# XuZerui2023/Radar-Signal-Simulation-and-Target-Detection

Measured on AMD Instinct MI355X. Metric: frames/sec + range-Doppler cells/sec, 16ch×8beam×4096samp×128pulse, higher is better.
Workload: dtype fp64 (complex128); 1 GPU; BASELINE config #2: x2 C=16 B=8 N=4096 P=128 G=2811; frames_per_launch=8, ring=8, parallelism=frame-sharded x1, used_samples=3027, targets_reported=258400

## Files before the change

include/rsp.h:

```cpp
#ifndef RSP_H
#define RSP_H

#include <stddef.h>
#include <stdint.h>

#ifdef __cplusplus
extern "C" {
#endif

#define RSP_ABI_VERSION 4

typedef enum rsp_status {
    RSP_OK = 0,
    RSP_ERR_INVALID = -1,
    RSP_ERR_UNSUPPORTED = -2,
    RSP_ERR_DEVICE = -3,
    RSP_ERR_NOMEM = -4,
    RSP_ERR_OVERFLOW = -5
} rsp_status;

typedef enum rsp_dtype {
    RSP_C64 = 1,
    RSP_C128 = 2
} rsp_dtype;
// ... 145 lines not shown
    int32_t Ls, ntaps, delay;
    int32_t Lh, M, V;
    int32_t nblocks;
    int32_t rows_per_wg;
} rsp_k2_segment;
typedef struct rsp_k2_layout {
    int32_t k2_pts;
    int32_t wg_per_cu;
    int32_t NZ;
    int32_t nseg, njobs;
    int32_t nwg;
    rsp_k2_segment seg[3];
} rsp_k2_layout;
int32_t rsp_query_k2_layout(const rsp_plan* plan, rsp_k2_layout* out);

int32_t rsp_plan_describe(const rsp_sig_config* cfg, const rsp_cfar_params* cfar,
                          const rsp_cluster_params* cluster, const rsp_precomputed* pre,
                          const rsp_plan_options* opt, int32_t ncu, rsp_sizes* sizes, rsp_k1_route* route);
int32_t rsp_plan_describe_k3(const rsp_sig_config* cfg, const rsp_cfar_params* cfar,
                             const rsp_cluster_params* cluster, const rsp_precomputed* pre,
                             const rsp_plan_options* opt, int32_t ncu, rsp_k3_tiling* tiling);
int32_t rsp_plan_describe_k2(const rsp_sig_config* cfg, const rsp_cfar_params* cfar,
                             const rsp_cluster_params* cluster, const rsp_precomputed* pre,
                             const rsp_plan_options* opt, int32_t ncu, rsp_k2_layout* layout);

int32_t rsp_process_cube(rsp_plan* plan, const void* cube, int32_t dtype, int32_t layout,
                         int32_t frame_idx, rsp_frame_out* out);

int32_t rsp_last_detections(const rsp_plan* plan, rsp_detection* dets, int32_t cap, int32_t* n);
int32_t rsp_last_targets(const rsp_plan* plan, rsp_target* targets, int32_t cap, int32_t* n);

int32_t rsp_process_targets(rsp_plan* plan, const rsp_target_in* targets, int32_t n_targets,
                            int32_t frame_idx, uint64_t seed, double p_noise, rsp_frame_out* out);

int32_t rsp_synthesize_device(rsp_plan* plan, const rsp_target_in* targets, int32_t n_targets,
                              int32_t frame_idx, uint64_t seed, double p_noise, void* d_cube);
int32_t rsp_profile_synthesis(rsp_plan* plan, const rsp_target_in* targets, int32_t n_targets, int32_t iters,
                              void* d_cube, float* ms_out, int64_t* bytes_out);

// ... 248 lines not shown
```

radar-signal-simulation-and-target-detection_amd/csrc/rsp_geometry.cpp:

```cpp
#include "rsp_geometry.h"

#include <algorithm>
#include <cmath>
#include <cstdint>
#include <utility>

__attribute__((visibility("hidden"))) int rsp_set_error(int code, const char* fmt, ...);

namespace {

template <class... A>
int fail(int code, const char* fmt, A... a) { return rsp_set_error(code, fmt, a...); }

using cd = std::complex<double>;

bool is_pow2(int x) { return x > 0 && (x & (x - 1)) == 0; }
int ilog2i(int x) { int l = 0; while ((1 << l) < x) ++l; return l; }
size_t cplx_bytes(const Geometry& g) { return g.prec == RSP_PREC_F64 ? 16 : 8; }

void fft_d(std::vector<cd>& a, int sign) {
    const int n = (int)a.size();
    if (!is_pow2(n)) {
        std::vector<cd> o(n);
        for (int k = 0; k < n; ++k) {
// ... 329 lines not shown
    for (const Unit& u : units) {
        int x = 0;
        for (int c = 1; c < 8; ++c)
            if (q[c].size() < q[x].size()) x = c;
        q[x].insert(q[x].end(), u.wgs.begin(), u.wgs.end());
    }
    std::vector<int>& order = h.k2order;
    size_t qmax = 0;
    for (auto& v : q) qmax = std::max(qmax, v.size());
    for (size_t sl = 0; sl < qmax; ++sl)
        for (int x = 0; x < 8; ++x)
            if (sl < q[x].size()) order.push_back(q[x][sl]);
    for (int w : single) order.push_back(w);
    if ((int)order.size() != g.nwg_k2)
        return fail(RSP_ERR_INVALID, "K2 dispatch order covers %d of %d workgroups", (int)order.size(), g.nwg_k2);
    return RSP_OK;
}

#define RSP_K3_TILE_KB 48
#define RSP_K3_RT_C128 32
int derive_k3_tiling(Geometry& g) {
    const size_t rsz = cplx_bytes(g) / 2;
    g.cfar_hR = (std::max(g.refR + g.guardR, 2) + 3) & ~3;
    g.cfar_RT = rsz == 4 ? 64 : RSP_K3_RT_C128;
    const bool k3_nohalo = k3_fast_params(g);
    const int hx = k3_nohalo ? 0 : 2;
    g.cfar_W = ((g.cfar_RT + hx * g.cfar_hR + 3) & ~3) + (rsz == 8 ? 2 : 0);
    const int hV = g.refV + g.guardV, ncut = std::max(g.P - 2 * hV, 1);
    const int hrows = k3_nohalo ? 0 : 2 * hV;
    const int rows_max = (int)((RSP_K3_TILE_KB * 1024) / ((size_t)g.cfar_W * rsz));
// ... 259 lines not shown
    return RSP_OK;
}

extern "C" int32_t rsp_plan_describe_k2(const rsp_sig_config* cfg, const rsp_cfar_params* cfar, const rsp_cluster_params* cluster,
                                        const rsp_precomputed* pre, const rsp_plan_options* opt, int32_t ncu,
                                        rsp_k2_layout* layout) {
    int rc = rsp_plan_check_args(cfg, cfar, cluster, pre, opt);
    if (rc) return rc;
    PlanHost h;
    if ((rc = rsp_plan_derive(cfg, cfar, cluster, pre, opt, ncu, &h))) return rc;
    const int32_t gates[RSP_MAX_SEG] = {pre->N_gate_narrow, pre->N_gate_medium, pre->N_gate_long};
    if (layout) rsp_fill_k2_layout(h.g, gates, layout);
    return RSP_OK;
}

int rsp_stage3_derive(int P, const int32_t* gates, const rsp_stage3_cfar_params* prm, S3Desc* out) {
    if (!gates || !prm || !out) return fail(RSP_ERR_INVALID, "null argument");
    const int64_t G = (int64_t)gates[0] + gates[1] + gates[2];
    if (P < 1 || gates[0] < 0 || gates[1] < 0 || gates[2] < 0 || G < 1 || G > INT32_MAX)
        return fail(RSP_ERR_INVALID, "bad map shape P=%d segments %d, %d, %d", P, gates[0], gates[1], gates[2]);
    const int r = prm->refCells_R, s = prm->saveCells_R;
    if (r < 1 || s < 0) return fail(RSP_ERR_INVALID, "bad CFAR window refCells_R=%d saveCells_R=%d (r >= 1, s >= 0)", r, s);
    if (prm->CFARmethod_R != 0 && prm->CFARmethod_R != 1)
        return fail(RSP_ERR_INVALID, "CFARmethod_R must be 0 (greatest of) or 1 (smallest of), got %d", prm->CFARmethod_R);
    if (prm->MTD_0v_num < 0) return fail(RSP_ERR_INVALID, "MTD_0v_num must be >= 0, got %d", prm->MTD_0v_num);
    if (!std::isfinite(prm->T_CFAR) || prm->T_CFAR <= 0) return fail(RSP_ERR_INVALID, "T_CFAR must be finite and > 0, got %g", prm->T_CFAR);
    const int64_t H = (int64_t)r + s;
    if (H > RSP_S3_HMAX)
        return fail(RSP_ERR_INVALID, "CFAR window refCells_R + saveCells_R = %lld exceeds the kernel's tile halo %d", (long long)H,
                    RSP_S3_HMAX);
// ... 86 lines not shown
```

radar-signal-simulation-and-target-detection_amd/csrc/rsp_geometry.h:

```cpp
#pragma once
#include "rsp.h"

#include <complex>
#include <stddef.h>
#include <stdint.h>
#include <vector>

#ifdef __HIPCC__
#define RSP_HD __host__ __device__
#else
#define RSP_HD
#endif

#define RSP_MAX_F 8
#define RSP_K2_POINTS 4096
#define RSP_K2_MIXPTS 2560
#define K1_THREADS 512

#define RSP_PREC_F32 0
#define RSP_PREC_F64 1

constexpr size_t RSP_LDS_BYTES = 160 * 1024;

struct SegDesc {
    int type;
    int ga, gb;
    int seg_lo;
    int lo, hi;
    int off;
    int ntaps, delay, Ls, taps_off;
    int Lh, M, logM, V, nblocks, H_off, tw_off;
    int rows_per_wg;
};

struct K2Job {
    int seg, blk, wg_begin, wg_count;
};

#define RSP_MAX_SEG 3
#define RSP_MAX_JOBS 16
#define RSP_MAX_IVL 4

struct Geometry {
    int prec;
    int C, B, P, N, G;
    int cpitch;
    int Gp;
    int NT, nU, ntiles, Ppad;
    int NZ, nzc;
    int twPp_elems;
    int pow2P, logP;
// ... 1 lines not shown
    int nseg, njobs, nwg_k2;
    int k2_pts;
    int cfar_RT, cfar_hR, cfar_W;
    int cfar_VB, cfar_nband, cfar_rows;
    int refR, guardR, refV, guardV;
    double T;
    int max_dets;
    int ncu;
    int k1_tiled;
    int mono_c;
    int nivl, ivl_lo[RSP_MAX_IVL], ivl_start[RSP_MAX_IVL];
    SegDesc segs[RSP_MAX_SEG];
    K2Job jobs[RSP_MAX_JOBS];
};
static_assert(sizeof(SegDesc) == 76 && sizeof(K2Job) == 16 && sizeof(Geometry) == 680, "kernel-argument layout");

RSP_HD inline bool k3_fast_params(const Geometry& g) {
    return g.refR == 5 && g.refV == 5 && g.guardR == 10 && g.guardV == 10 && (g.cfar_RT == 32 || g.cfar_RT == 64);
}

RSP_HD inline int k3_ntiles(const Geometry& g) {
    const int rc0 = g.refR + g.guardR;
    return (g.G - rc0 - (rc0 & ~3) + g.cfar_RT - 1) / g.cfar_RT;
}

RSP_HD inline long long k3_map_bytes(const Geometry& g, int real_bytes) {
    if (k3_fast_params(g)) {
        const int hV = g.refV + g.guardV, c0 = (g.refR + g.guardR) & ~3;
        const int rows = g.P - 2 * hV > 0 ? g.P - 2 * hV : 0;
        const int c1 = c0 + k3_ntiles(g) * g.cfar_RT < g.G ? c0 + k3_ntiles(g) * g.cfar_RT : g.G;
// ... 98 lines not shown
size_t mtd_cols_lds(const Geometry& g);

struct PlanHost {
    typedef std::complex<double> cd;
    Geometry g{};
    std::vector<SegDesc> segs;
    std::vector<K2Job> jobs;
    int det_bound = 1;
    size_t z_elems = 0, rdm_elems = 0, mag_elems = 0;
    std::vector<double> atab;
    std::vector<cd> twP, twPp, twD, twQ;
    std::vector<double> win, taps;
    std::vector<cd> H, twM;
    std::vector<double> range_axis, velocity_axis, beam_angles, klut;
    std::vector<int> k2order;
};

#define RSP_S3_CH 256
#define RSP_S3_ROWS 16
#define RSP_S3_HMAX 64
struct S3Desc {
    int P, G;
    int seg_a[3], seg_n[3];
    int r, s, H;
    int method;
    int z0, z1;
    double T;
};
int rsp_stage3_derive(int P, const int32_t* gates, const rsp_stage3_cfar_params* prm, S3Desc* out);

// ... 6 lines not shown
    int method;
    double T;
};
RSP_HD constexpr size_t vc_lds_bytes(int halo, size_t rs) { return (size_t)(RSP_VC_ROWS + 2 * halo) * RSP_VC_COLS * rs; }
int rsp_vcfar_derive(int P, int G, const rsp_vcfar_params* prm, VcDesc* out);

int rsp_plan_check_args(const rsp_sig_config* cfg, const rsp_cfar_params* cfar, const rsp_cluster_params* cluster,
                        const rsp_precomputed* pre, const rsp_plan_options* opt);
int rsp_plan_derive(const rsp_sig_config* cfg, const rsp_cfar_params* cfar, const rsp_cluster_params* cluster,
                    const rsp_precomputed* pre, const rsp_plan_options* opt, int ncu, PlanHost* out);

void rsp_fill_sizes(const Geometry& g, int det_bound, rsp_sizes* s);
void rsp_fill_k1_route(const Geometry& g, rsp_k1_route* out);
void rsp_fill_k3_tiling(const Geometry& g, rsp_k3_tiling* out);
void rsp_fill_k2_layout(const Geometry& g, const int32_t gates[RSP_MAX_SEG], rsp_k2_layout* out);
```

radar-signal-simulation-and-target-detection_amd/csrc/rsp_internal.h:

```cpp
#pragma once
#include <hip/hip_runtime.h>
#include <stdint.h>

#include "rsp_geometry.h"
#include "rsp_music_geometry.h"

#define RSP_LANES 4
#define RSP_NLANES 3
#define K2_THREADS 256
#define RSP_THREADS 256

__device__ __forceinline__ void rsp_philox10(uint32_t c[4], uint32_t k0, uint32_t k1) {
    const uint32_t M0 = 0xD2511F53u, M1 = 0xCD9E8D57u;
#pragma unroll
    for (int r = 0; r < 10; ++r) {
        const uint64_t p0 = (uint64_t)M0 * c[0];
        const uint64_t p1 = (uint64_t)M1 * c[2];
        const uint32_t hi0 = (uint32_t)(p0 >> 32), lo0 = (uint32_t)p0;
        const uint32_t hi1 = (uint32_t)(p1 >> 32), lo1 = (uint32_t)p1;
        const uint32_t n0 = hi1 ^ c[1] ^ k0, n2 = hi0 ^ c[3] ^ k1;
        c[0] = n0; c[1] = lo1; c[2] = n2; c[3] = lo0;
        k0 += 0x9E3779B9u;
        k1 += 0xBB67AE85u;
    }
// ... 13 lines not shown
    unsigned long long* trace;
    DevDet* dets[RSP_MAX_F];
    int* count[RSP_MAX_F];
};

struct DevConsts {
    const void* Atab;
    const void* win;
    const void* twP;
    const void* twPp;
    const void* twD;
    const void* twQ;
    const void* taps;
    const void* H;
    const void* twM;
    const int* k2order;
    const double* range_axis;
    const double* velocity_axis;
    const double* beam_angles;
    const double* klut;
    double deltaR, deltaV;
};

hipError_t launch_k1(const Geometry& g, const DevConsts& k, const FramePtrs& fp, int nf, int mode, hipStream_t s);
hipError_t launch_stream_copy(const void* in, void* out, size_t n16, int ncu, hipStream_t s);
hipError_t launch_k2(const Geometry& g, const DevConsts& k, const FramePtrs& fp, int nf, int rows, hipStream_t s);
hipError_t launch_k3(const Geometry& g, const DevConsts& k, const FramePtrs& fp, int nf, hipStream_t s);
hipError_t launch_mtd_cols(const Geometry& g, const DevConsts& k, const void* pc, void* rdm, hipStream_t s);
hipError_t launch_synth(const Geometry& g, const double* tx, const SynthTargets& tg, int nt, void* tab, int frame_idx,
                        uint64_t seed, double noise_scale, void* cube, hipStream_t s);
hipError_t launch_s3(const S3Desc& d, int prec, bool cplx, const void* in, int n_maps, double* amp, double* thr,
// ... 9 lines not shown
```

radar-signal-simulation-and-target-detection_amd/csrc/rsp_kernels.hip:

```cpp
#include "rsp_internal.h"
#include "rsp_cmag.h"
#include "rsp_noise_math.h"
#include <math.h>
#include <algorithm>

namespace {

typedef float f32x4 __attribute__((ext_vector_type(4)));
typedef double f64x4 __attribute__((ext_vector_type(4)));
typedef unsigned int u32x2 __attribute__((ext_vector_type(2)));
typedef unsigned int u32x4 __attribute__((ext_vector_type(4)));

template <class T> struct CxT;
template <> struct CxT<float> { typedef f2 V; };
template <> struct CxT<double> { typedef d2 V; };
template <class T> using cx = typename CxT<T>::V;
template <class V> struct ScalT;
template <> struct ScalT<f2> { typedef float S; };
template <> struct ScalT<d2> { typedef double S; };
template <class V> using scal = typename ScalT<V>::S;

__device__ __forceinline__ f2 vmul(f2 a, f2 b) { return a.xx * b + a.yy * f2{-b.y, b.x}; }
__device__ __forceinline__ d2 vmul(d2 a, d2 b) { return d2{a.x * b.x - a.y * b.y, a.x * b.y + a.y * b.x}; }
template <bool INV>
// ... 221 lines not shown
template <bool INV, class V> struct Dft<12, INV, V> {
    static __device__ __forceinline__ void run(V* a) { dft_pfa<4, 3, INV>(a); }
};

template <int SH>
__device__ __forceinline__ int lidx(int i) { return SH ? i + (i >> SH) : i; }

template <class V>
struct StoreLds {
    V* buf;
    __device__ __forceinline__ void put(int, int, int, int loff, V x) const { buf[loff] = x; }
};
template <class St> struct StoresLds { static constexpr bool value = false; };
template <class V> struct StoresLds<StoreLds<V>> { static constexpr bool value = true; };

template <int R, bool INV, bool CMP, int NS, class V, class TW>
__device__ __forceinline__ void load_tw(const TW& twk, V (&w)[R]) {
    if constexpr (!CMP) {
#pragma unroll
        for (int r = 1; r < R; ++r) {
            const V t = twk[r - 1];
            w[r] = V{t.x, INV ? -t.y : t.y};
        }
    } else {
        constexpr int lgR = clog2(R - 1) + 1;
        V b[lgR];
#pragma unroll
        for (int i = 0; i < lgR; ++i) {
            const V t = twk[i * NS];
            b[i] = V{t.x, INV ? -t.y : t.y};
        }
#pragma unroll
        for (int r = 1; r < R; ++r) {
            const int hb = 1 << clog2(r);
            w[r] = (hb == r) ? b[clog2(r)] : vmul(w[hb], w[r - hb]);
        }
    }
}

template <int SH, int D, int R>
constexpr bool lidx_sep() {
    constexpr int p = 1 << SH;
    return SH == 0 || D % p == 0 || (p % D == 0 && ((D * R) % p == 0 || p % (D * R) == 0));
}
template <int SH, int D>
constexpr int lidx_off(int r) {
    return r * D + (SH ? (r * D) >> SH : 0);
}

template <int R, bool INV, int NB, int SH, int NTHR, int L, int NS, bool CMP = false, int XL = 0, class V, class TW>
__device__ __forceinline__ void sh_load(const V* buf, int rs, int nrows, const TW& tw, V (&v)[NB][R],
// ... 2 lines not shown
    static_assert(!XL || nb % 128 == 0, "XOR-swizzled input needs r nb to keep the swizzle bits");
    constexpr bool SEP = lidx_sep<SH, nb, R>();
    const int total = nb * nrows;
#pragma unroll
    for (int t = 0; t < NB; ++t) {
        const int beta = tix + t * NTHR;
        if (beta < total) {
            const int row = beta / nb, j = beta - row * nb;
            const V* src = XL ? buf + row * L + (j ^ ((j >> 4) & 7)) : buf + row * rs + (SEP ? lidx<SH>(j) : 0);
            V w[R];
            if (NS > 1) load_tw<R, INV, CMP, NS>(tw + (CMP ? j % NS : (j % NS) * tw_row(R, CMP)), w);
#pragma unroll
            for (int r = 0; r < R; ++r) {
                V x = XL ? src[r * nb] : (SEP ? src[lidx_off<SH, nb>(r)] : src[lidx<SH>(j + r * nb)]);
                if (r > 0 && NS > 1) x = vmul(x, w[r]);
                v[t][r] = x;
            }
        }
    }
}

template <int R, bool INV, int NB, int SH, int NTHR, int L, int NS, int XL = 0, class V, class St>
__device__ __forceinline__ void sh_store(V (&v)[NB][R], int rs, int nrows, const St& st, int tix = threadIdx.x) {
    constexpr int nb = L / R;
    static_assert(!XL || (NS == 1 && R == 16), "XOR-swizzled output: Ns = 1 radix-16 passes");
    const int total = nb * nrows;
#pragma unroll
    for (int t = 0; t < NB; ++t) {
        const int beta = tix + t * NTHR;
        if (beta < total) {
// ... 795 lines not shown
}

template <class T> constexpr int k2_sh() { return RSP_K2_SH; }
constexpr int K2_NOPAD_SH = 30;
template <class T, bool NOPAD> constexpr int k2_sh_np() { return NOPAD ? K2_NOPAD_SH : k2_sh<T>(); }

constexpr int k2_tw_lds(RadixPlan p) {
    return plan_tw_total(p, true) + (plan_is_palindrome(p) ? 0 : plan_tw_total(plan_rev(p), true));
}
constexpr int k2_tw_lds_max() {
    int m = k2_tw_lds(plan_os_2560());
    for (int lg = 6; lg <= 11; ++lg) m = k2_tw_lds(plan_os_pow2(lg)) > m ? k2_tw_lds(plan_os_pow2(lg)) : m;
    return m;
}

template <class T, int SH>
__device__ __forceinline__ void k2_epilogue(const cx<T>* L, int rs, int rows, int row0, int rows_total, int Lh1, int g0,
                                            int gend, cx<T>* __restrict__ rdm, T* __restrict__ mag, int G, int Gp) {
    typedef cx<T> V;
    const int nkeep = gend - g0;
    for (int r = 0; r < rows; ++r) {
        const int rho = row0 + r;
        if (rho >= rows_total) break;
        const V* src = L + r * rs + Lh1;
        const int pad0 = SH ? Lh1 : 0;
        const __amdgpu_buffer_rsrc_t mr = buf_rsrc(mag + (size_t)rho * Gp + g0, (unsigned)nkeep * (unsigned)sizeof(T));
        if (rdm) {
            const __amdgpu_buffer_rsrc_t rr = buf_rsrc(rdm + (size_t)rho * G + g0, (unsigned)nkeep * (unsigned)sizeof(V));
            for (int e = threadIdx.x; e < nkeep; e += K2_THREADS) {
                const V x = src[e + (SH ? ((pad0 + e) >> SH) : 0)];
                buf_st<RSP_RDM_AUX>(rr, (unsigned)e * (unsigned)sizeof(V), x);
                buf_st1(mr, (unsigned)e * (unsigned)sizeof(T), cmag(x));
            }
        } else {
            for (int e = threadIdx.x; e < nkeep; e += K2_THREADS)
                buf_st1(mr, (unsigned)e * (unsigned)sizeof(T), cmag(src[e + (SH ? ((pad0 + e) >> SH) : 0)]));
        }
    }
}

template <int R, int S, class V>
__device__ __forceinline__ void k2_apply_h(V (&x)[R], __amdgpu_buffer_rsrc_t hr, int j) {
    asm volatile("" ::: "memory");
    V h[R];
#pragma unroll
    for (int r = 0; r < R; ++r) h[r] = buf_ld<V>(hr, (unsigned)(j + r * S) * (unsigned)sizeof(V));
#pragma unroll
    for (int r = 0; r < R; ++r) x[r] = vmul(x[r], h[r]);
}

template <bool LDS, class V>
// ... 161 lines not shown
    if (tid < nb0 * rows) {
        const ZWin zw = zrow_window(g, z, row0 + rl, rows_total, off, lo, hi);
        k2_load_wrow<nb0>(g, zw, a + j - lo + off, v0[0]);
        if constexpr (!EPI) {
            const __amdgpu_buffer_rsrc_t hr = buf_rsrc(H + sd.H_off, (unsigned)(M * sizeof(V)));
#pragma unroll
            for (int r = 0; r < R0; ++r)
                hreg[0][r] = buf_ld<V>(hr, (unsigned)(j + r * nb0) * (unsigned)sizeof(V));
        }
    }
    V* twL = L + k2_lds_data(g.k2_pts, SH);
    if constexpr (!NOPAD) stage_lds<K2_THREADS>(twL, twl, NTWF);
    const auto twF = k2_tw_src<!NOPAD, V>(twL, twl);
    const auto twI = twF;
    constexpr int XZ = R0 == 16 ? 1 : 0;
    sh_store<R0, false, NB0, SH, K2_THREADS, M, 1, XZ>(v0, rs, rows, StoreLds<V>{L}, tid);
    __syncthreads();
    K2_STAMP(1);
    sh_pass<R1, false, NB1, SH, K2_THREADS, M, NS1, CMP, XZ>(L, rs, rows, twF, StoreLds<V>{L});
    K2_STAMP(2);
    {
        V v[NB0][R0];
        sh_load<R0, false, NB0, SH, K2_THREADS, M, NS2, CMP>(L, rs, rows, twF + TW2, v, tid);
        __syncthreads();
        const __amdgpu_buffer_rsrc_t hr = buf_rsrc(H + sd.H_off, (unsigned)(M * sizeof(V)));
#pragma unroll
        for (int t = 0; t < NB0; ++t) {
            Dft<R0, false, V>::run(v[t]);
            if constexpr (EPI) {
                k2_apply_h<R0, nb0>(v[t], hr, j);
            } else {
#pragma unroll
                for (int r = 0; r < R0; ++r) v[t][r] = vmul(v[t][r], hreg[t][r]);
            }
        }
        sh_store<R0, true, NB0, SH, K2_THREADS, M, 1, XZ>(v, rs, rows, StoreLds<V>{L}, tid);
        __syncthreads();
    }
    K2_STAMP(3);
    sh_pass<R1, true, NB1, SH, K2_THREADS, M, NS1, CMP, XZ>(L, rs, rows, twI, StoreLds<V>{L});
    K2_STAMP(4);
    const int gend = min(sd.gb, g0 + sd.V);
    if constexpr (EPI) {
        sh_pass<R0, true, NB0, SH, K2_THREADS, M, NS2, CMP>(L, rs, rows, twI + TW2, StoreLds<V>{L});
        k2_epilogue<T, SH>(L, rs, rows, row0, rows_total, Lh1, g0, gend, rdm, mag, G, g.Gp);
    } else {
        static_assert(EPI || (rows == 1 && NS2 == nb0), "last pass: thread j's outputs are j + r NS2 of one row");
        V v[NB0][R0];
        sh_load<R0, true, NB0, SH, K2_THREADS, M, NS2, CMP>(L, rs, rows, twI + TW2, v, tid);
        if (rdm)
            sh_store<R0, true, NB0, SH, K2_THREADS, M, NS2>(
                v, rs, rows, StoreRowK<V, true, NS2, R0>(rdm, mag, G, g.Gp, row0, rows_total, Lh1, g0, gend), tid);
        else
            sh_store<R0, true, NB0, SH, K2_THREADS, M, NS2>(
                v, rs, rows, StoreRowK<V, false, NS2, R0>(rdm, mag, G, g.Gp, row0, rows_total, Lh1, g0, gend), tid);
    }
}

template <class T, int WGS>
__global__ __launch_bounds__(K2_THREADS, WGS) void k2_pc(Geometry g, DevConsts k, FramePtrs fp, int rows_total) {
    constexpr bool EPI = WGS >= 3;
    constexpr bool NOPAD = WGS == 4;
    typedef cx<T> V;
    V* L = reinterpret_cast<V*>(rsp_lds);
    const int f = blockIdx.y;
    const int wg = k.k2order[blockIdx.x];
    int ji = 0;
    while (ji + 1 < g.njobs && wg >= g.jobs[ji + 1].wg_begin) ++ji;
    const K2Job job = g.jobs[ji];
    const SegDesc& sd = g.segs[job.seg];
    const int rows = sd.rows_per_wg;
    const int row0 = (wg - job.wg_begin) * rows;
    const V* __restrict__ z = static_cast<const V*>(fp.z[f]);
    V* __restrict__ rdm = static_cast<V*>(fp.rdm[f]);
    T* __restrict__ mag = static_cast<T*>(fp.mag[f]);
    const int P = g.P, G = g.G;
    const int lo = sd.lo, hi = sd.hi, off = sd.off;
    const int tid = threadIdx.x;
    K2_STAMP(0);
    K2_TAG((unsigned long long)(sd.type * 16 + sd.logM));

    if (sd.type == 1 && sd.logM == 0) {
        k2_fft_job_mix<T, 2560, 16, 10, EPI, NOPAD>(g, k, sd, job, z, rdm, mag, row0, rows_total, L);
    } else if (sd.type == 1) {
        constexpr int PTS = WGS >= 3 ? 2048 : RSP_K2_POINTS;
        constexpr int LGTOP = WGS >= 3 ? 11 : 12;
        switch (sd.logM) {
// ... 814 lines not shown
```

radar-signal-simulation-and-target-detection_amd/csrc/rsp_plan.cpp:

```cpp
#include "rsp.h"
#include "rsp_frame_host.h"
#include "rsp_internal.h"

#include <algorithm>
#include <cmath>
#include <complex>
#include <cstdarg>
#include <cstdio>
#include <cstring>
#include <cstdlib>
#include <condition_variable>
#include <deque>
#include <functional>
#include <memory>
#include <mutex>
#include <string>
#include <thread>
#include <vector>

__attribute__((visibility("hidden"))) void rsp_cluster_frame(const rsp_cluster_params& cp, std::vector<rsp_detection>& dets,
                                                             std::vector<rsp_target>& final_targets);

namespace {

// ... 98 lines not shown
    DevConsts k{};
    rsp_cluster_params cl{};
    SynthConsts sc{};
    int F = 1;
    int det_bound = 1;
    size_t esz = 16;
    size_t rsz = 8;
    size_t z_elems = 0, rdm_elems = 0, mag_elems = 0;
    std::vector<void*> dev_allocs;
    double* d_tx = nullptr;
    double* d_stab = nullptr;
    void* d_cube = nullptr;
    void* d_aux = nullptr;
    void* d_smap = nullptr;
    int32_t gates[3] = {0, 0, 0};
    bool aux_valid = false;
    struct DevBuf {
        void* p = nullptr;
        size_t cap = 0;
    };
    DevBuf s3_in, s3_amp, s3_thr, s3_flags, s3_hits, s3_count;
    unsigned char* h_stage = nullptr;
    size_t h_stage_bytes = 0;
    Lane lanes[RSP_LANES];
    int nlanes = RSP_NLANES;
    int next_lane = 0;
    bool time_stages = false;
    double stage_ms[3] = {0, 0, 0};
    int64_t stage_launches = 0, stage_frames = 0;
    const void* pend_in[RSP_MAX_F];
// ... 541 lines not shown
    rsp_plan* p = new rsp_plan();
    auto bail = [&](int rc) { delete p; return rc; };
    p->device = device;
    p->F = opt->frames_per_launch;
    p->cl = *cluster;
    p->sc = SynthConsts{cfg->c, cfg->fs, cfg->wavelength, cfg->element_spacing, cfg->prt, pre->P_signal_unscaled};
    p->esz = opt->precision == RSP_C128 ? 16 : 8;
    p->rsz = p->esz / 2;
    p->g = h.g;
    p->det_bound = h.det_bound;
    p->z_elems = h.z_elems; p->rdm_elems = h.rdm_elems; p->mag_elems = h.mag_elems;
    p->gates[0] = pre->N_gate_narrow; p->gates[1] = pre->N_gate_medium; p->gates[2] = pre->N_gate_long;

    DevConsts& k = p->k;
    double *dra, *dva, *dang, *dkl;
    int* dord;
    if ((rc = p->upload_r(&k.Atab, h.atab)) || (rc = p->upload_c(&k.twP, h.twP)) || (rc = p->upload_c(&k.twPp, h.twPp)) ||
        (rc = p->upload_c(&k.twD, h.twD)) || (rc = p->upload_c(&k.twQ, h.twQ)) || (rc = p->upload_r(&k.win, h.win)) ||
        (rc = p->upload_r(&k.taps, h.taps)) || (rc = p->upload_c(&k.H, h.H)) || (rc = p->upload_c(&k.twM, h.twM)) ||
        (rc = p->upload(&dra, h.range_axis)) || (rc = p->upload(&dva, h.velocity_axis)) ||
        (rc = p->upload(&dang, h.beam_angles)) || (rc = p->upload(&dkl, h.klut)) || (rc = p->upload(&dord, h.k2order)))
        return bail(rc);
    k.range_axis = dra; k.velocity_axis = dva; k.beam_angles = dang; k.klut = dkl;
    k.k2order = dord;
    k.deltaR = pre->deltaR; k.deltaV = pre->deltaV;
    const Geometry& g = p->g;
    if (pre->tx_pulse) {
        std::vector<double> tx(pre->tx_pulse, pre->tx_pulse + 2 * (size_t)g.N);
        if ((rc = p->upload(&p->d_tx, tx))) return bail(rc);
    }
    if ((rc = p->dalloc(&p->d_stab, (size_t)2 * RSP_MAX_SYNTH_TARGETS * (g.P + g.C)))) return bail(rc);
    if ((rc = p->dalloc_bytes(&p->d_cube, (size_t)std::max(g.C, g.B) * g.cpitch * p->esz))) return bail(rc);
    for (auto& L : p->lanes)
        if ((rc = setup_lane(p, L))) return bail(rc);
    *out = p;
    return RSP_OK;
}

int32_t rsp_set_stage_timing(rsp_plan* p, int32_t on) {
// ... 27 lines not shown
    if (!p || !out) return fail(RSP_ERR_INVALID, "null argument");
    rsp_fill_k1_route(p->g, out);
    return RSP_OK;
}

int32_t rsp_query_k3_tiling(const rsp_plan* p, rsp_k3_tiling* out) {
    if (!p || !out) return fail(RSP_ERR_INVALID, "null argument");
    rsp_fill_k3_tiling(p->g, out);
    return RSP_OK;
}

int32_t rsp_query_k2_layout(const rsp_plan* p, rsp_k2_layout* out) {
    if (!p || !out) return fail(RSP_ERR_INVALID, "null argument");
    rsp_fill_k2_layout(p->g, p->gates, out);
    return RSP_OK;
}

int32_t rsp_process_cube(rsp_plan* p, const void* cube, int32_t dtype, int32_t layout, int32_t frame_idx,
                         rsp_frame_out* out) {
    if (!p || !cube) return fail(RSP_ERR_INVALID, "null argument");
    if (layout != RSP_LAYOUT_PNC) return fail(RSP_ERR_UNSUPPORTED, "layout %d", layout);
    HIPCHK(hipSetDevice(p->device));
    int rc = drain_all(p);
    if (rc) return rc;
    if ((rc = upload_cube(p, cube, dtype, p->g.C, p->d_cube, p->lanes[0].stream))) return rc;
    return run_sync_frame(p, p->d_cube, frame_idx, out);
}

static int synth_into(rsp_plan* p, const rsp_target_in* t, int nt, int frame_idx, uint64_t seed, double p_noise,
                      void* d_cube, hipStream_t s, bool sync) {
// ... 521 lines not shown
```

radar-signal-simulation-and-target-detection_amd/rsp/_abi.py:

```python
import ctypes as ct
import os

LIB_PATH = os.path.join(os.path.dirname(os.path.abspath(__file__)), 'librsp.so')
_INTREE = LIB_PATH

RSP_OK, RSP_ERR_INVALID, RSP_ERR_UNSUPPORTED, RSP_ERR_DEVICE, RSP_ERR_NOMEM, RSP_ERR_OVERFLOW = 0, -1, -2, -3, -4, -5
RSP_C64, RSP_C128 = 1, 2
RSP_LAYOUT_PNC = 0

_dp = ct.POINTER(ct.c_double)


class SigConfig(ct.Structure):
    _fields_ = [('c', ct.c_double), ('fs', ct.c_double), ('fc', ct.c_double), ('prt', ct.c_double),
                ('wavelength', ct.c_double), ('element_spacing', ct.c_double),
                ('prtNum', ct.c_int32), ('point_PRT', ct.c_int32), ('channel_num', ct.c_int32),
                ('beam_num', ct.c_int32)]


class CfarParams(ct.Structure):
    _fields_ = [('refCells_V', ct.c_int32), ('guardCells_V', ct.c_int32), ('refCells_R', ct.c_int32),
                ('guardCells_R', ct.c_int32), ('T_CFAR', ct.c_double)]


# ... 49 lines not shown


class K3Tiling(ct.Structure):
    _fields_ = [('fast', ct.c_int32), ('RT', ct.c_int32), ('hR', ct.c_int32), ('W', ct.c_int32),
                ('n_tiles', ct.c_int32), ('n_bands', ct.c_int32), ('VB', ct.c_int32), ('rows', ct.c_int32)]


class K2Segment(ct.Structure):
    _fields_ = [(n, ct.c_int32) for n in ('present', 'type', 'ga', 'gb', 'seg_lo', 'lo', 'hi', 'Ls', 'ntaps', 'delay',
                                          'Lh', 'M', 'V', 'nblocks', 'rows_per_wg')]


class K2Layout(ct.Structure):
    _fields_ = [('k2_pts', ct.c_int32), ('wg_per_cu', ct.c_int32), ('NZ', ct.c_int32), ('nseg', ct.c_int32),
                ('njobs', ct.c_int32), ('nwg', ct.c_int32), ('seg', K2Segment * 3)]


class Stage3CfarParams(ct.Structure):
    _fields_ = [('refCells_R', ct.c_int32), ('saveCells_R', ct.c_int32), ('CFARmethod_R', ct.c_int32),
                ('MTD_0v_num', ct.c_int32), ('T_CFAR', ct.c_double)]


class Stage3Hit(ct.Structure):
    _fields_ = [('v_idx', ct.c_int32), ('r_idx', ct.c_int32), ('beam_idx', ct.c_int32), ('reserved', ct.c_int32),
                ('amp', ct.c_double), ('threshold', ct.c_double)]


class Stage3Info(ct.Structure):
    _fields_ = [('P', ct.c_int32), ('G', ct.c_int32), ('seg_first', ct.c_int32 * 3), ('seg_len', ct.c_int32 * 3),
                ('notch_first', ct.c_int32), ('notch_last', ct.c_int32), ('halo', ct.c_int32),
# ... 94 lines not shown
    'rsp_plan_options_default': (ct.c_int32, [ct.POINTER(PlanOptions)]),
    'rsp_plan_destroy': (ct.c_int32, [_P]),
    'rsp_query_sizes': (ct.c_int32, [_P, ct.POINTER(Sizes)]),
    'rsp_query_k1_route': (ct.c_int32, [_P, ct.POINTER(K1Route)]),
    'rsp_plan_describe': (ct.c_int32, [ct.POINTER(SigConfig), ct.POINTER(CfarParams), ct.POINTER(ClusterParams),
                                       ct.POINTER(Precomputed), ct.POINTER(PlanOptions), ct.c_int32, ct.POINTER(Sizes),
                                       ct.POINTER(K1Route)]),
    'rsp_query_k3_tiling': (ct.c_int32, [_P, ct.POINTER(K3Tiling)]),
    'rsp_plan_describe_k3': (ct.c_int32, [ct.POINTER(SigConfig), ct.POINTER(CfarParams), ct.POINTER(ClusterParams),
                                          ct.POINTER(Precomputed), ct.POINTER(PlanOptions), ct.c_int32,
                                          ct.POINTER(K3Tiling)]),
    'rsp_query_k2_layout': (ct.c_int32, [_P, ct.POINTER(K2Layout)]),
    'rsp_plan_describe_k2': (ct.c_int32, [ct.POINTER(SigConfig), ct.POINTER(CfarParams), ct.POINTER(ClusterParams),
                                          ct.POINTER(Precomputed), ct.POINTER(PlanOptions), ct.c_int32,
                                          ct.POINTER(K2Layout)]),
    'rsp_process_cube': (ct.c_int32, [_P, _P, ct.c_int32, ct.c_int32, ct.c_int32, ct.POINTER(FrameOut)]),
    'rsp_process_targets': (ct.c_int32, [_P, ct.POINTER(TargetIn), ct.c_int32, ct.c_int32, ct.c_uint64,
                                         ct.c_double, ct.POINTER(FrameOut)]),
    'rsp_synthesize_device': (ct.c_int32, [_P, ct.POINTER(TargetIn), ct.c_int32, ct.c_int32, ct.c_uint64,
                                           ct.c_double, _P]),
    'rsp_profile_synthesis': (ct.c_int32, [_P, ct.POINTER(TargetIn), ct.c_int32, ct.c_int32, _P,
                                           ct.POINTER(ct.c_float), ct.POINTER(ct.c_int64)]),
    'rsp_enqueue_device': (ct.c_int32, [_P, _P, ct.c_int32]),
    'rsp_enqueue_device_n': (ct.c_int32, [_P, ct.POINTER(_P), ct.POINTER(ct.c_int32), ct.c_int32]),
    'rsp_enqueue_device_rdm': (ct.c_int32, [_P, _P, ct.c_int32, _P]),
    'rsp_enqueue_device_rdm_n': (ct.c_int32, [_P, ct.POINTER(_P), ct.POINTER(ct.c_int32), ct.POINTER(_P), ct.c_int32]),
    'rsp_enqueue_host': (ct.c_int32, [_P, _P, ct.c_int32, ct.c_int32]),
    'rsp_host_alloc': (ct.c_int32, [_P, ct.c_int64, ct.POINTER(_P)]),
    'rsp_host_free': (ct.c_int32, [_P, _P]),
    'rsp_process_targets_multi': (ct.c_int32, [ct.POINTER(_P), ct.c_int32, ct.POINTER(ct.POINTER(TargetIn)),
# ... 110 lines not shown
```

radar-signal-simulation-and-target-detection_amd/rsp/plan.py:

```python
import ctypes as ct
import numpy as np

from . import _abi
from ._abi import check, lib


def _dptr(a):
    return a.ctypes.data_as(ct.POINTER(ct.c_double))


def _complex_arg(a):
    c64 = np.asarray(a).dtype == np.complex64
    a = np.asfortranarray(a, None if c64 else np.complex128)
    return a, a.ctypes.data_as(ct.c_void_p), _abi.RSP_C64 if c64 else _abi.RSP_C128


def _gate_cols_arg(gate_cols):
    return (ct.c_int32 * 6)(*[int(x) for fl in gate_cols for x in fl])


def _with_hits(call, first_cap, hits_cap, want_hits):
    cap = (int(hits_cap) if hits_cap is not None else first_cap) if want_hits else 0
    hits = np.zeros(max(cap, 1), HIT_DTYPE)
    total = call(cap, hits.ctypes.data_as(ct.POINTER(_abi.Stage3Hit)) if cap else None, True)
# ... 102 lines not shown
    segs = [{k: getattr(s, k) for k, _ in _abi.K2Segment._fields_ if k != 'present'} if s.present else None
            for s in L.seg]
    return dict(k2_pts=L.k2_pts, wg_per_cu=L.wg_per_cu, NZ=L.NZ, nseg=L.nseg, njobs=L.njobs, nwg=L.nwg, segments=segs)


def describe_k2(config, cfar_params, cluster_params, precomputed_data, precision='c128', k1_tiled=False, ncu=256):
    keep = []
    cfg, cfar, cluster, pre = _marshal(config, cfar_params, cluster_params, precomputed_data, keep)
    opt = _options(0, 1, precision, k1_tiled, 'amplitude')
    L = _abi.K2Layout()
    check(lib().rsp_plan_describe_k2(ct.byref(cfg), ct.byref(cfar), ct.byref(cluster), ct.byref(pre), ct.byref(opt),
                                     int(ncu), ct.byref(L)))
    return _k2_dict(L)


HIT_DTYPE = np.dtype([('v_idx', np.int32), ('r_idx', np.int32), ('beam_idx', np.int32), ('reserved', np.int32),
                      ('amp', np.float64), ('threshold', np.float64)])
STAGE3_WANT = ('mtd', 'amp', 'flags', 'threshold', 'hits')


def _stage3_params(cfar):
    return _abi.Stage3CfarParams(refCells_R=int(cfar['refCells_R']), saveCells_R=int(cfar['saveCells_R']),
                                 CFARmethod_R=int(cfar['CFARmethod_R']), MTD_0v_num=int(cfar['MTD_0v_num']),
                                 T_CFAR=float(cfar['T_CFAR']))


def describe_stage3(P, segments, cfar):
    n1, n2, n3 = (int(x) for x in segments)
    cfg = _abi.SigConfig(prtNum=int(P))
    pre = _abi.Precomputed(N_gate_narrow=n1, N_gate_medium=n2, N_gate_long=n3, N_total_gate=n1 + n2 + n3)
# ... 57 lines not shown

    def k1_route(self):
        r = _abi.K1Route()
        check(lib().rsp_query_k1_route(self.h, ct.byref(r)))
        return _route_dict(r)

    def k3_tiling(self):
        t = _abi.K3Tiling()
        check(lib().rsp_query_k3_tiling(self.h, ct.byref(t)))
        return _tiling_dict(t)

    def k2_layout(self):
        L = _abi.K2Layout()
        check(lib().rsp_query_k2_layout(self.h, ct.byref(L)))
        return _k2_dict(L)

    def _frame_out(self, want_rdm, want_cfar):
        o = _abi.FrameOut()
        bufs = {}
        if want_rdm:
            bufs['rdm'] = np.empty((self.P, self.G, self.B), np.complex128, order='F')
            o.rdm = bufs['rdm'].ctypes.data_as(ct.POINTER(ct.c_double))
        if want_cfar and self.B > 1:
            bufs['cfar'] = np.empty((self.P, self.G, self.B - 1), np.float64, order='F')
            o.cfar_maps = _dptr(bufs['cfar'])
        o.dets, o.dets_cap, o.targets, o.targets_cap = None, 0, None, 0
        return o, bufs, None, None

    def last_detections(self):
        n = ct.c_int32()
# ... 352 lines not shown
```

Baseline: 17850 frames/s.

## Precompute K2 workgroup records, prefetch twiddles across barriers, unroll epilogue stores

K2's per-workgroup job lookup, which walked the job table, is replaced by a host-precomputed 16-byte record (segment, block, first row) read once per workgroup. In the no-pad path, twiddle base values for the next FFT pass are fetched from global memory before the preceding LDS store and barrier, then expanded in registers, so the loads overlap the sync. The epilogue loop that writes magnitudes and RDM is unrolled by four, with loads batched ahead of stores. These raise register pressure through the held twiddle buffers and add query APIs for the records.

```diff
diff --git a/include/rsp.h b/include/rsp.h
--- a/include/rsp.h
+++ b/include/rsp.h
@@ -183,6 +183,14 @@
 } rsp_k2_layout;
 int32_t rsp_query_k2_layout(const rsp_plan* plan, rsp_k2_layout* out);
 
+typedef struct rsp_k2_record {
+    int32_t seg;
+    int32_t blk;
+    int32_t row0;
+    int32_t wg;
+} rsp_k2_record;
+int32_t rsp_query_k2_records(const rsp_plan* plan, rsp_k2_record* out, int32_t cap, int32_t* n);
+
 int32_t rsp_plan_describe(const rsp_sig_config* cfg, const rsp_cfar_params* cfar,
                           const rsp_cluster_params* cluster, const rsp_precomputed* pre,
                           const rsp_plan_options* opt, int32_t ncu, rsp_sizes* sizes, rsp_k1_route* route);
@@ -192,6 +200,10 @@
 int32_t rsp_plan_describe_k2(const rsp_sig_config* cfg, const rsp_cfar_params* cfar,
                              const rsp_cluster_params* cluster, const rsp_precomputed* pre,
                              const rsp_plan_options* opt, int32_t ncu, rsp_k2_layout* layout);
+int32_t rsp_plan_describe_k2_records(const rsp_sig_config* cfg, const rsp_cfar_params* cfar,
+                                     const rsp_cluster_params* cluster, const rsp_precomputed* pre,
+                                     const rsp_plan_options* opt, int32_t ncu, rsp_k2_record* out, int32_t cap,
+                                     int32_t* n);
 
 int32_t rsp_process_cube(rsp_plan* plan, const void* cube, int32_t dtype, int32_t layout,
                          int32_t frame_idx, rsp_frame_out* out);
diff --git a/radar-signal-simulation-and-target-detection_amd/csrc/rsp_geometry.cpp b/radar-signal-simulation-and-target-detection_amd/csrc/rsp_geometry.cpp
--- a/radar-signal-simulation-and-target-detection_amd/csrc/rsp_geometry.cpp
+++ b/radar-signal-simulation-and-target-detection_amd/csrc/rsp_geometry.cpp
@@ -367,6 +367,13 @@
     for (int w : single) order.push_back(w);
     if ((int)order.size() != g.nwg_k2)
         return fail(RSP_ERR_INVALID, "K2 dispatch order covers %d of %d workgroups", (int)order.size(), g.nwg_k2);
+    h.k2rec.reserve(order.size());
+    for (int wg : order) {
+        size_t ji = 0;
+        while (ji + 1 < h.jobs.size() && wg >= h.jobs[ji + 1].wg_begin) ++ji;
+        const K2Job& jb = h.jobs[ji];
+        h.k2rec.push_back(K2Rec{jb.seg, jb.blk, (wg - jb.wg_begin) * h.segs[jb.seg].rows_per_wg, wg});
+    }
     return RSP_OK;
 }
 
@@ -656,6 +663,25 @@
     return RSP_OK;
 }
 
+int rsp_fill_k2_records(const std::vector<K2Rec>& rec, rsp_k2_record* out, int32_t cap, int32_t* n) {
+    if (cap < 0 || (cap > 0 && !out)) return fail(RSP_ERR_INVALID, "bad record buffer (capacity %d)", cap);
+    const size_t m = std::min((size_t)cap, rec.size());
+    for (size_t i = 0; i < m; ++i) out[i] = rsp_k2_record{rec[i].seg, rec[i].blk, rec[i].row0, rec[i].wg};
+    if (n) *n = (int32_t)rec.size();
+    return RSP_OK;
+}
+
+extern "C" int32_t rsp_plan_describe_k2_records(const rsp_sig_config* cfg, const rsp_cfar_params* cfar,
+                                                const rsp_cluster_params* cluster, const rsp_precomputed* pre,
+                                                const rsp_plan_options* opt, int32_t ncu, rsp_k2_record* out, int32_t cap,
+                                                int32_t* n) {
+    int rc = rsp_plan_check_args(cfg, cfar, cluster, pre, opt);
+    if (rc) return rc;
+    PlanHost h;
+    if ((rc = rsp_plan_derive(cfg, cfar, cluster, pre, opt, ncu, &h))) return rc;
+    return rsp_fill_k2_records(h.k2rec, out, cap, n);
+}
+
 int rsp_stage3_derive(int P, const int32_t* gates, const rsp_stage3_cfar_params* prm, S3Desc* out) {
     if (!gates || !prm || !out) return fail(RSP_ERR_INVALID, "null argument");
     const int64_t G = (int64_t)gates[0] + gates[1] + gates[2];
diff --git a/radar-signal-simulation-and-target-detection_amd/csrc/rsp_geometry.h b/radar-signal-simulation-and-target-detection_amd/csrc/rsp_geometry.h
--- a/radar-signal-simulation-and-target-detection_amd/csrc/rsp_geometry.h
+++ b/radar-signal-simulation-and-target-detection_amd/csrc/rsp_geometry.h
@@ -35,6 +35,10 @@
 
 struct K2Job {
     int seg, blk, wg_begin, wg_count;
+};
+
+struct K2Rec {
+    int seg, blk, row0, wg;
 };
 
 #define RSP_MAX_SEG 3
@@ -66,6 +70,7 @@
     K2Job jobs[RSP_MAX_JOBS];
 };
 static_assert(sizeof(SegDesc) == 76 && sizeof(K2Job) == 16 && sizeof(Geometry) == 680, "kernel-argument layout");
+static_assert(sizeof(K2Rec) == 16, "one 16-byte scalar load per workgroup");
 
 RSP_HD inline bool k3_fast_params(const Geometry& g) {
     return g.refR == 5 && g.refV == 5 && g.guardR == 10 && g.guardV == 10 && (g.cfar_RT == 32 || g.cfar_RT == 64);
@@ -194,6 +199,7 @@
     std::vector<cd> H, twM;
     std::vector<double> range_axis, velocity_axis, beam_angles, klut;
     std::vector<int> k2order;
+    std::vector<K2Rec> k2rec;
 };
 
 #define RSP_S3_CH 256
@@ -230,3 +236,4 @@
 void rsp_fill_k1_route(const Geometry& g, rsp_k1_route* out);
 void rsp_fill_k3_tiling(const Geometry& g, rsp_k3_tiling* out);
 void rsp_fill_k2_layout(const Geometry& g, const int32_t gates[RSP_MAX_SEG], rsp_k2_layout* out);
+int rsp_fill_k2_records(const std::vector<K2Rec>& rec, rsp_k2_record* out, int32_t cap, int32_t* n);
diff --git a/radar-signal-simulation-and-target-detection_amd/csrc/rsp_internal.h b/radar-signal-simulation-and-target-detection_amd/csrc/rsp_internal.h
--- a/radar-signal-simulation-and-target-detection_amd/csrc/rsp_internal.h
+++ b/radar-signal-simulation-and-target-detection_amd/csrc/rsp_internal.h
@@ -51,7 +51,7 @@
     const void* taps;
     const void* H;
     const void* twM;
-    const int* k2order;
+    const K2Rec* k2rec;
     const double* range_axis;
     const double* velocity_axis;
     const double* beam_angles;
diff --git a/radar-signal-simulation-and-target-detection_amd/csrc/rsp_kernels.hip b/radar-signal-simulation-and-target-detection_amd/csrc/rsp_kernels.hip
--- a/radar-signal-simulation-and-target-detection_amd/csrc/rsp_kernels.hip
+++ b/radar-signal-simulation-and-target-detection_amd/csrc/rsp_kernels.hip
@@ -259,6 +259,20 @@
 template <class St> struct StoresLds { static constexpr bool value = false; };
 template <class V> struct StoresLds<StoreLds<V>> { static constexpr bool value = true; };
 
+template <int R, int NS, class V, class TW>
+__device__ __forceinline__ void tw_fetch(const TW& twk, V (&b)[tw_row(R, true)]) {
+#pragma unroll
+    for (int i = 0; i < tw_row(R, true); ++i) b[i] = twk[i * NS];
+}
+template <int R, bool INV, class V>
+__device__ __forceinline__ void tw_expand(const V (&b)[tw_row(R, true)], V (&w)[R]) {
+#pragma unroll
+    for (int r = 1; r < R; ++r) {
+        const int hb = 1 << clog2(r);
+        const V t = b[clog2(r)];
+        w[r] = (hb == r) ? V{t.x, INV ? -t.y : t.y} : vmul(w[hb], w[r - hb]);
+    }
+}
 template <int R, bool INV, bool CMP, int NS, class V, class TW>
 __device__ __forceinline__ void load_tw(const TW& twk, V (&w)[R]) {
     if constexpr (!CMP) {
@@ -268,18 +282,9 @@
             w[r] = V{t.x, INV ? -t.y : t.y};
         }
     } else {
-        constexpr int lgR = clog2(R - 1) + 1;
-        V b[lgR];
-#pragma unroll
-        for (int i = 0; i < lgR; ++i) {
-            const V t = twk[i * NS];
-            b[i] = V{t.x, INV ? -t.y : t.y};
-        }
-#pragma unroll
-        for (int r = 1; r < R; ++r) {
-            const int hb = 1 << clog2(r);
-            w[r] = (hb == r) ? b[clog2(r)] : vmul(w[hb], w[r - hb]);
-        }
+        V b[tw_row(R, true)];
+        tw_fetch<R, NS>(twk, b);
+        tw_expand<R, INV>(b, w);
     }
 }
 
@@ -312,6 +317,42 @@
             for (int r = 0; r < R; ++r) {
                 V x = XL ? src[r * nb] : (SEP ? src[lidx_off<SH, nb>(r)] : src[lidx<SH>(j + r * nb)]);
                 if (r > 0 && NS > 1) x = vmul(x, w[r]);
+                v[t][r] = x;
+            }
+        }
+    }
+}
+
+template <int R, int NB, int NTHR, int L, int NS, class V, class TW>
+__device__ __forceinline__ void sh_tw_fetch(int nrows, const TW& tw, V (&b)[NB][tw_row(R, true)], int tix = threadIdx.x) {
+    constexpr int nb = L / R;
+    static_assert(NS > 1, "a pass with twiddles");
+    const int total = nb * nrows;
+#pragma unroll
+    for (int t = 0; t < NB; ++t) {
+        const int beta = tix + t * NTHR;
+        if (beta < total) tw_fetch<R, NS>(tw + (beta % nb) % NS, b[t]);
+    }
+}
+template <int R, bool INV, int NB, int SH, int NTHR, int L, int NS, int XL = 0, class V>
+__device__ __forceinline__ void sh_load_pf(const V* buf, int rs, int nrows, const V (&b)[NB][tw_row(R, true)],
+                                           V (&v)[NB][R], int tix = threadIdx.x) {
+    constexpr int nb = L / R;
+    static_assert(!XL || nb % 128 == 0, "XOR-swizzled input needs r nb to keep the swizzle bits");
+    constexpr bool SEP = lidx_sep<SH, nb, R>();
+    const int total = nb * nrows;
+#pragma unroll
+    for (int t = 0; t < NB; ++t) {
+        const int beta = tix + t * NTHR;
+        if (beta < total) {
+            const int row = beta / nb, j = beta - row * nb;
+            const V* src = XL ? buf + row * L + (j ^ ((j >> 4) & 7)) : buf + row * rs + (SEP ? lidx<SH>(j) : 0);
+            V w[R];
+            tw_expand<R, INV>(b[t], w);
+#pragma unroll
+            for (int r = 0; r < R; ++r) {
+                V x = XL ? src[r * nb] : (SEP ? src[lidx_off<SH, nb>(r)] : src[lidx<SH>(j + r * nb)]);
+                if (r > 0) x = vmul(x, w[r]);
                 v[t][r] = x;
             }
         }
@@ -1137,6 +1178,40 @@
     return m;
 }
 
+template <class T, int SH, int U, bool RDM>
+__device__ __forceinline__ void k2_epi_trip(const cx<T>* src, int pad0, int e0, int nkeep, __amdgpu_buffer_rsrc_t rr,
+                                            __amdgpu_buffer_rsrc_t mr) {
+    typedef cx<T> V;
+    V x[U];
+#pragma unroll
+    for (int u = 0; u < U; ++u) {
+        const int i = min(e0 + u * K2_THREADS, nkeep - 1);
+        x[u] = src[i + (SH ? ((pad0 + i) >> SH) : 0)];
+    }
+    T m[U];
+#pragma unroll
+    for (int u = 0; u < U; ++u) m[u] = cmag(x[u]);
+#pragma unroll
+    for (int u = 0; u < U; ++u) {
+        const unsigned e = (unsigned)(e0 + u * K2_THREADS);
+        if (RDM) buf_st<RSP_RDM_AUX>(rr, e * (unsigned)sizeof(V), x[u]);
+        buf_st1(mr, e * (unsigned)sizeof(T), m[u]);
+    }
+}
+template <class T, int SH, bool RDM>
+__device__ __forceinline__ void k2_epi_row(const cx<T>* src, int pad0, int nkeep, __amdgpu_buffer_rsrc_t rr,
+                                           __amdgpu_buffer_rsrc_t mr) {
+    constexpr int U = 4;
+    int e0 = threadIdx.x, left = nkeep;
+    for (; left > (U - 1) * K2_THREADS; left -= U * K2_THREADS, e0 += U * K2_THREADS)
+        k2_epi_trip<T, SH, U, RDM>(src, pad0, e0, nkeep, rr, mr);
+    if (left > 2 * K2_THREADS)
+        k2_epi_trip<T, SH, 3, RDM>(src, pad0, e0, nkeep, rr, mr);
+    else if (left > K2_THREADS)
+        k2_epi_trip<T, SH, 2, RDM>(src, pad0, e0, nkeep, rr, mr);
+    else if (left > 0)
+        k2_epi_trip<T, SH, 1, RDM>(src, pad0, e0, nkeep, rr, mr);
+}
 template <class T, int SH>
 __device__ __forceinline__ void k2_epilogue(const cx<T>* L, int rs, int rows, int row0, int rows_total, int Lh1, int g0,
                                             int gend, cx<T>* __restrict__ rdm, T* __restrict__ mag, int G, int Gp) {
@@ -1150,14 +1225,9 @@
         const __amdgpu_buffer_rsrc_t mr = buf_rsrc(mag + (size_t)rho * Gp + g0, (unsigned)nkeep * (unsigned)sizeof(T));
         if (rdm) {
             const __amdgpu_buffer_rsrc_t rr = buf_rsrc(rdm + (size_t)rho * G + g0, (unsigned)nkeep * (unsigned)sizeof(V));
-            for (int e = threadIdx.x; e < nkeep; e += K2_THREADS) {
-                const V x = src[e + (SH ? ((pad0 + e) >> SH) : 0)];
-                buf_st<RSP_RDM_AUX>(rr, (unsigned)e * (unsigned)sizeof(V), x);
-                buf_st1(mr, (unsigned)e * (unsigned)sizeof(T), cmag(x));
-            }
+            k2_epi_row<T, SH, true>(src, pad0, nkeep, rr, mr);
         } else {
-            for (int e = threadIdx.x; e < nkeep; e += K2_THREADS)
-                buf_st1(mr, (unsigned)e * (unsigned)sizeof(T), cmag(src[e + (SH ? ((pad0 + e) >> SH) : 0)]));
+            k2_epi_row<T, SH, false>(src, pad0, nkeep, mr, mr);
         }
     }
 }
@@ -1349,10 +1419,20 @@
     const auto twF = k2_tw_src<!NOPAD, V>(twL, twl);
     const auto twI = twF;
     constexpr int XZ = R0 == 16 ? 1 : 0;
+    V b1[NOPAD ? NB1 : 1][tw_row(R1, true)], b2[NOPAD ? NB0 : 1][tw_row(R0, true)];
+    if constexpr (NOPAD) sh_tw_fetch<R1, NB1, K2_THREADS, M, NS1>(rows, twF, b1, tid);
     sh_store<R0, false, NB0, SH, K2_THREADS, M, 1, XZ>(v0, rs, rows, StoreLds<V>{L}, tid);
     __syncthreads();
     K2_STAMP(1);
-    sh_pass<R1, false, NB1, SH, K2_THREADS, M, NS1, CMP, XZ>(L, rs, rows, twF, StoreLds<V>{L});
+    if constexpr (NOPAD) {
+        V v[NB1][R1];
+        sh_load_pf<R1, false, NB1, SH, K2_THREADS, M, NS1, XZ>(L, rs, rows, b1, v, tid);
+        __syncthreads();
+        sh_store<R1, false, NB1, SH, K2_THREADS, M, NS1>(v, rs, rows, StoreLds<V>{L}, tid);
+        __syncthreads();
+    } else {
+        sh_pass<R1, false, NB1, SH, K2_THREADS, M, NS1, CMP, XZ>(L, rs, rows, twF, StoreLds<V>{L});
+    }
     K2_STAMP(2);
     {
         V v[NB0][R0];
@@ -1373,10 +1453,27 @@
         __syncthreads();
     }
     K2_STAMP(3);
-    sh_pass<R1, true, NB1, SH, K2_THREADS, M, NS1, CMP, XZ>(L, rs, rows, twI, StoreLds<V>{L});
+    if constexpr (NOPAD) {
+        V v[NB1][R1];
+        sh_load<R1, true, NB1, SH, K2_THREADS, M, NS1, CMP, XZ>(L, rs, rows, twI, v, tid);
+        asm volatile("" ::: "memory");
+        sh_tw_fetch<R0, NB0, K2_THREADS, M, NS2>(rows, twI + TW2, b2, tid);
+        __syncthreads();
+        sh_store<R1, true, NB1, SH, K2_THREADS, M, NS1>(v, rs, rows, StoreLds<V>{L}, tid);
+        __syncthreads();
+    } else {
+        sh_pass<R1, true, NB1, SH, K2_THREADS, M, NS1, CMP, XZ>(L, rs, rows, twI, StoreLds<V>{L});
+    }
     K2_STAMP(4);
     const int gend = min(sd.gb, g0 + sd.V);
-    if constexpr (EPI) {
+    if constexpr (EPI && NOPAD) {
+        V v[NB0][R0];
+        sh_load_pf<R0, true, NB0, SH, K2_THREADS, M, NS2>(L, rs, rows, b2, v, tid);
+        __syncthreads();
+        sh_store<R0, true, NB0, SH, K2_THREADS, M, NS2>(v, rs, rows, StoreLds<V>{L}, tid);
+        __syncthreads();
+        k2_epilogue<T, SH>(L, rs, rows, row0, rows_total, Lh1, g0, gend, rdm, mag, G, g.Gp);
+    } else if constexpr (EPI) {
         sh_pass<R0, true, NB0, SH, K2_THREADS, M, NS2, CMP>(L, rs, rows, twI + TW2, StoreLds<V>{L});
         k2_epilogue<T, SH>(L, rs, rows, row0, rows_total, Lh1, g0, gend, rdm, mag, G, g.Gp);
     } else {
@@ -1399,13 +1496,11 @@
     typedef cx<T> V;
     V* L = reinterpret_cast<V*>(rsp_lds);
     const int f = blockIdx.y;
-    const int wg = k.k2order[blockIdx.x];
-    int ji = 0;
-    while (ji + 1 < g.njobs && wg >= g.jobs[ji + 1].wg_begin) ++ji;
-    const K2Job job = g.jobs[ji];
-    const SegDesc& sd = g.segs[job.seg];
+    const K2Rec rec = k.k2rec[blockIdx.x];
+    const K2Job job{rec.seg, rec.blk, 0, 0};
+    const SegDesc& sd = g.segs[rec.seg];
     const int rows = sd.rows_per_wg;
-    const int row0 = (wg - job.wg_begin) * rows;
+    const int row0 = rec.row0;
     const V* __restrict__ z = static_cast<const V*>(fp.z[f]);
     V* __restrict__ rdm = static_cast<V*>(fp.rdm[f]);
     T* __restrict__ mag = static_cast<T*>(fp.mag[f]);
diff --git a/radar-signal-simulation-and-target-detection_amd/csrc/rsp_plan.cpp b/radar-signal-simulation-and-target-detection_amd/csrc/rsp_plan.cpp
--- a/radar-signal-simulation-and-target-detection_amd/csrc/rsp_plan.cpp
+++ b/radar-signal-simulation-and-target-detection_amd/csrc/rsp_plan.cpp
@@ -136,6 +136,7 @@
     void* d_aux = nullptr;
     void* d_smap = nullptr;
     int32_t gates[3] = {0, 0, 0};
+    std::vector<K2Rec> k2rec;
     bool aux_valid = false;
     struct DevBuf {
         void* p = nullptr;
@@ -707,15 +708,16 @@
 
     DevConsts& k = p->k;
     double *dra, *dva, *dang, *dkl;
-    int* dord;
+    K2Rec* drec;
     if ((rc = p->upload_r(&k.Atab, h.atab)) || (rc = p->upload_c(&k.twP, h.twP)) || (rc = p->upload_c(&k.twPp, h.twPp)) ||
         (rc = p->upload_c(&k.twD, h.twD)) || (rc = p->upload_c(&k.twQ, h.twQ)) || (rc = p->upload_r(&k.win, h.win)) ||
         (rc = p->upload_r(&k.taps, h.taps)) || (rc = p->upload_c(&k.H, h.H)) || (rc = p->upload_c(&k.twM, h.twM)) ||
         (rc = p->upload(&dra, h.range_axis)) || (rc = p->upload(&dva, h.velocity_axis)) ||
-        (rc = p->upload(&dang, h.beam_angles)) || (rc = p->upload(&dkl, h.klut)) || (rc = p->upload(&dord, h.k2order)))
+        (rc = p->upload(&dang, h.beam_angles)) || (rc = p->upload(&dkl, h.klut)) || (rc = p->upload(&drec, h.k2rec)))
         return bail(rc);
     k.range_axis = dra; k.velocity_axis = dva; k.beam_angles = dang; k.klut = dkl;
-    k.k2order = dord;
+    k.k2rec = drec;
+    p->k2rec = std::move(h.k2rec);
     k.deltaR = pre->deltaR; k.deltaV = pre->deltaV;
     const Geometry& g = p->g;
     if (pre->tx_pulse) {
@@ -773,6 +775,11 @@
     if (!p || !out) return fail(RSP_ERR_INVALID, "null argument");
     rsp_fill_k2_layout(p->g, p->gates, out);
     return RSP_OK;
+}
+
+int32_t rsp_query_k2_records(const rsp_plan* p, rsp_k2_record* out, int32_t cap, int32_t* n) {
+    if (!p) return fail(RSP_ERR_INVALID, "null argument");
+    return rsp_fill_k2_records(p->k2rec, out, cap, n);
 }
 
 int32_t rsp_process_cube(rsp_plan* p, const void* cube, int32_t dtype, int32_t layout, int32_t frame_idx,
diff --git a/radar-signal-simulation-and-target-detection_amd/rsp/_abi.py b/radar-signal-simulation-and-target-detection_amd/rsp/_abi.py
--- a/radar-signal-simulation-and-target-detection_amd/rsp/_abi.py
+++ b/radar-signal-simulation-and-target-detection_amd/rsp/_abi.py
@@ -87,6 +87,10 @@
 class K2Layout(ct.Structure):
     _fields_ = [('k2_pts', ct.c_int32), ('wg_per_cu', ct.c_int32), ('NZ', ct.c_int32), ('nseg', ct.c_int32),
                 ('njobs', ct.c_int32), ('nwg', ct.c_int32), ('seg', K2Segment * 3)]
+
+
+class K2Record(ct.Structure):
+    _fields_ = [(n, ct.c_int32) for n in ('seg', 'blk', 'row0', 'wg')]
 
 
 class Stage3CfarParams(ct.Structure):
@@ -211,6 +215,11 @@
     'rsp_plan_describe_k2': (ct.c_int32, [ct.POINTER(SigConfig), ct.POINTER(CfarParams), ct.POINTER(ClusterParams),
                                           ct.POINTER(Precomputed), ct.POINTER(PlanOptions), ct.c_int32,
                                           ct.POINTER(K2Layout)]),
+    'rsp_query_k2_records': (ct.c_int32, [_P, ct.POINTER(K2Record), ct.c_int32, ct.POINTER(ct.c_int32)]),
+    'rsp_plan_describe_k2_records': (ct.c_int32, [ct.POINTER(SigConfig), ct.POINTER(CfarParams),
+                                                  ct.POINTER(ClusterParams), ct.POINTER(Precomputed),
+                                                  ct.POINTER(PlanOptions), ct.c_int32, ct.POINTER(K2Record), ct.c_int32,
+                                                  ct.POINTER(ct.c_int32)]),
     'rsp_process_cube': (ct.c_int32, [_P, _P, ct.c_int32, ct.c_int32, ct.c_int32, ct.POINTER(FrameOut)]),
     'rsp_process_targets': (ct.c_int32, [_P, ct.POINTER(TargetIn), ct.c_int32, ct.c_int32, ct.c_uint64,
                                          ct.c_double, ct.POINTER(FrameOut)]),
diff --git a/radar-signal-simulation-and-target-detection_amd/rsp/plan.py b/radar-signal-simulation-and-target-detection_amd/rsp/plan.py
--- a/radar-signal-simulation-and-target-detection_amd/rsp/plan.py
+++ b/radar-signal-simulation-and-target-detection_amd/rsp/plan.py
@@ -140,6 +140,26 @@
     return _k2_dict(L)
 
 
+K2_RECORD_FIELDS = ('seg', 'blk', 'row0', 'wg')
+
+
+def _k2_records(call):
+    n = ct.c_int32(0)
+    check(call(None, 0, ct.byref(n)))
+    rec = (_abi.K2Record * max(n.value, 1))()
+    check(call(rec, n.value, ct.byref(n)))
+    return np.array([[getattr(r, f) for f in K2_RECORD_FIELDS] for r in rec[:n.value]], dtype=np.int32).reshape(-1, 4)
+
+
+def describe_k2_records(config, cfar_params, cluster_params, precomputed_data, precision='c128', k1_tiled=False,
+                        ncu=256):
+    keep = []
+    cfg, cfar, cluster, pre = _marshal(config, cfar_params, cluster_params, precomputed_data, keep)
+    opt = _options(0, 1, precision, k1_tiled, 'amplitude')
+    return _k2_records(lambda out, cap, n: lib().rsp_plan_describe_k2_records(
+        ct.byref(cfg), ct.byref(cfar), ct.byref(cluster), ct.byref(pre), ct.byref(opt), int(ncu), out, cap, n))
+
+
 HIT_DTYPE = np.dtype([('v_idx', np.int32), ('r_idx', np.int32), ('beam_idx', np.int32), ('reserved', np.int32),
                       ('amp', np.float64), ('threshold', np.float64)])
 STAGE3_WANT = ('mtd', 'amp', 'flags', 'threshold', 'hits')
@@ -227,6 +247,9 @@
         L = _abi.K2Layout()
         check(lib().rsp_query_k2_layout(self.h, ct.byref(L)))
         return _k2_dict(L)
+
+    def k2_records(self):
+        return _k2_records(lambda out, cap, n: lib().rsp_query_k2_records(self.h, out, cap, n))
 
     def _frame_out(self, want_rdm, want_cfar):
         o = _abi.FrameOut()
```

After: 18070 frames/s (median of 6 runs). 1.2% higher.
